# Zhen-Dong/HAWQ

Hardware: NVIDIA H100
Metric: images/sec ResNet-50 W8A8 & W4A4 @batch128, 1/2/4/8xH100; % int-TC roofline (higher is better)
Workload: dtype int8

## Files before the change

hawq_b200/csrc/conv_igemm.cuh:

```cuda
#pragma once
#include <type_traits>

#include "common.cuh"
#include "wgmma.cuh"

namespace hawq {

struct ConvParams {
  const uint8_t* x;
  const int8_t* w;
  const hawq_chan* chan;
  const void* res;
  const hawq_chan* res_chan;
  const float* fscale;
  void* out;
  void* out_low;
  int32_t* status;
  int N, H, W, Cin, Cout, KH, KW, stride, pad, Ho, Wo, M, K;
  int cin_chunks;
  int x_pix_bytes;
  int mode, relu, out_bits, lo, hi;
  int res_kind, res_bits;
  uint32_t res_m;
  int res_e;
  int y_bits, low_bits;
  uint32_t low_m;
  int low_e, low_lo, low_hi;
  int cout_store;
  int scalar_over_one;
  int scalar_unchecked;
  int check_ovf;
  int bias_lo, bias_hi;
  const uint8_t* x2;
  const int8_t* w2;
  int H2, W2, stride2, cin_chunks2, x2_pix_bytes;
};

constexpr int CONV_BM = 128;
constexpr int CONV_STAGES = 4;
constexpr int CONV_THREADS = 256;

template <int BN>
struct ChanSmem {
  static constexpr int M_OFF = BN * (int)sizeof(hawq_chan);
  static constexpr int M1_OFF = M_OFF + BN * 8;
  static constexpr int RC_OFF = M1_OFF + BN * 8;
  static constexpr int CB_OFF = RC_OFF + BN * (int)sizeof(hawq_chan);
  static constexpr int BYTES = CB_OFF + BN * 8;
  hawq_chan* chan;
  double* M;
  double* M1;
  hawq_chan* rc;
  double* Cb;
  __device__ explicit ChanSmem(uint8_t* base)
      : chan(reinterpret_cast<hawq_chan*>(base)), M(reinterpret_cast<double*>(base + M_OFF)),
        M1(reinterpret_cast<double*>(base + M1_OFF)), rc(reinterpret_cast<hawq_chan*>(base + RC_OFF)),
        Cb(reinterpret_cast<double*>(base + CB_OFF)) {}
};

template <int BN, bool A4>
struct ConvSmem {
  static constexpr int A_ROW = A4 ? 32 : 64;
  static constexpr int A_STAGE = CONV_BM * A_ROW;
  static constexpr int B_STAGE = BN * 64;
  static constexpr int PIPE = CONV_STAGES * (A_STAGE + B_STAGE);
  static constexpr int OUT_PITCH = BN + 16;
  static constexpr int OUT_STAGE = CONV_BM * OUT_PITCH;
  static constexpr int RES16 = CONV_BM * (BN * 2 + 16);
  static constexpr int RES32 = CONV_BM * (BN * 4 + 32);
  static constexpr int RES16_OFF = PIPE;
  static constexpr int RES32_OFF = OUT_STAGE;
  static constexpr int MAIN = PIPE + RES16 > RES32_OFF + RES32 ? PIPE + RES16 : RES32_OFF + RES32;
  static constexpr int CHAN_OFF = MAIN;
  static constexpr int TOTAL = CHAN_OFF + ChanSmem<BN>::BYTES;
  static_assert(OUT_STAGE <= PIPE, "the low-bit staging tile must fit in the freed ring");
  static_assert(2 * (TOTAL + 1024) <= 228 * 1024, "two CTAs per SM must fit in shared memory");
};

template <int ROW_BYTES>
__device__ __forceinline__ int swz(int row, int ch) {
  if constexpr (ROW_BYTES == 64) return row * 64 + ((ch ^ ((row >> 1) & 3)) << 4);
  else return row * 32 + ((ch ^ ((row >> 2) & 1)) << 4);
}

constexpr int FAM_REQUANT = 0, FAM_RESIDUAL = 1, FAM_STORE = 2, FAM_REQUANT_CAPPED = 3;

template <bool CLAMPED>
struct RqFp64 {
  bool checked;
  bool ovf = false;
  static constexpr double kMagic = 6755399441055744.0;
  __device__ static double acc_bias(int32_t acc, double cb, int32_t) {
    const double d = __hiloint2double(0x43300000, acc ^ 0x80000000) - cb;
    return CLAMPED ? fmin(fmax(d, -2147483648.0), 2147483647.0) : d;
  }
  __device__ static double of_i32(int32_t v) {
    return __hiloint2double(0x43300000, v ^ 0x80000000) - 4503601774854144.0;
  }
  __device__ static double of_u16(uint32_t u) { return __hiloint2double(0x43300000, (int)u) - 4503599627370496.0; }
  __device__ int32_t term(double d, double M, uint32_t, int32_t, bool count) {
    const double t = __fma_rn(d, M, kMagic);
    if (checked && count) {
      const double q = t - kMagic;
      ovf |= q > 2147483647.0 || q < -2147483648.0;
    }
    return __double2loint(t);
  }
};
struct RqExact {
  bool checked;
  bool ovf = false;
  __device__ static int32_t acc_bias(int32_t acc, double, int32_t bias) { return sat_add(acc, bias); }
  __device__ static int32_t of_i32(int32_t v) { return v; }
  __device__ static int32_t of_u16(uint32_t u) { return (int32_t)u; }
  __device__ int32_t term(int32_t v, double, uint32_t m, int32_t e, bool count) {
    const long long q = rhe_requant64(v, m, e);
    if (checked && count) ovf |= q > 2147483647ll || q < -2147483648ll;
    return sat_i32(q);
  }
};

struct RqPolicy {
  bool over_one;
  bool unchecked;
  bool clamped;
};

template <int BN, bool RESIDUAL, bool CAPS = false>
__device__ RqPolicy load_channel_block(const ConvParams& p, int n0, const ChanSmem<BN>& cs) {
  int over_one = p.scalar_over_one, unchecked = p.scalar_unchecked, bias_out = 0;
  const int tid = threadIdx.x;
  if (tid < BN) {
    hawq_chan c = p.chan[n0 + tid];
    if (CAPS) c.reserved = p.relu == 2 ? min(p.hi, c.reserved) : p.hi;
    cs.chan[tid] = c;
    cs.M[tid] = dyadic_to_double(c.m, c.e);
    cs.Cb[tid] = 4503601774854144.0 - (double)c.bias;
    bias_out = c.bias < p.bias_lo || c.bias > p.bias_hi;
    over_one |= !dyadic_is_fast(c.m, c.e);
    unchecked |= !dyadic_is_wide(c.m, c.e);
    if (RESIDUAL && p.res_kind == 1) {
      const hawq_chan rc = p.res_chan[n0 + tid];
      cs.rc[tid] = rc;
      cs.M1[tid] = dyadic_to_double(rc.m, rc.e);
      over_one |= !dyadic_is_fast(rc.m, rc.e);
      unchecked |= !dyadic_is_wide(rc.m, rc.e);
    }
  }
  RqPolicy pol;
  pol.over_one = __syncthreads_or(over_one) != 0;
  pol.unchecked = __syncthreads_or(unchecked) != 0;
  pol.clamped = __syncthreads_or(bias_out) != 0;
  return pol;
}

template <bool RESIDUAL, class F>
__device__ __forceinline__ void with_rq(const RqPolicy& pol, const ConvParams& p, F&& f) {
  const bool fp64 = !pol.over_one || (RESIDUAL && p.check_ovf && !pol.unchecked);
  if (!fp64) f(RqExact{RESIDUAL && p.check_ovf != 0});
  else if (pol.clamped) f(RqFp64<true>{RESIDUAL && pol.over_one});
  else f(RqFp64<false>{RESIDUAL && pol.over_one});
}

template <class Rq>
__device__ __forceinline__ int32_t residual_y(Rq& rq, int32_t res_term, int32_t acc, double cb, const int4& c, double M, bool ok,
                                              int32_t relu_floor) {
  return max(sat_add(res_term, rq.term(rq.acc_bias(acc, cb, c.x), M, c.y, c.z, ok)), relu_floor);
}
template <class Rq>
__device__ __forceinline__ int32_t residual_low(Rq& rq, int32_t y, double low_M, const ConvParams& p) {
  return clampi(rq.term(rq.of_i32(y), low_M, p.low_m, p.low_e, false), p.low_lo, p.low_hi);
}
__device__ __forceinline__ uint32_t stream16_pair(int32_t y0, int32_t y1, bool ok, int& ymax) {
  if (ok) ymax = max(ymax, max(y0, y1));
  return (uint32_t)min(y0, 65535) | ((uint32_t)min(y1, 65535) << 16);
}
__device__ __forceinline__ void residual_flags(const ConvParams& p, int ymax, bool ovf) {
  if (ymax > 65535) atomicOr(p.status, HAWQ_FLAG_RESIDUAL_OVERFLOW);
  if (ovf) atomicOr(p.status, HAWQ_FLAG_REQUANT_OVERFLOW);
}
__device__ __forceinline__ void stage_low_pair(uint8_t* s, int pitch, int row, int col, int q0, int q1) {
  *reinterpret_cast<uint16_t*>(s + row * pitch + col) = (uint16_t)__byte_perm(q0, q1, 0x0040);
}

__device__ __forceinline__ void copy_out_rows(const uint8_t* s, int s_pitch, uint8_t* g, size_t g_pitch, int row_bytes, int m0, int M) {
  const int cpr = row_bytes / 16;
  for (int id = threadIdx.x; id < CONV_BM * cpr; id += blockDim.x) {
    const int row = id / cpr, j = id - row * cpr;
    if (m0 + row < M)
      *reinterpret_cast<int4*>(g + (size_t)(m0 + row) * g_pitch + j * 16) = *reinterpret_cast<const int4*>(s + row * s_pitch + j * 16);
  }
}
template <int BN>
__device__ __forceinline__ void copy_out_low(const uint8_t* s, int pitch, uint8_t* gout, int bits, int m0, int n0, int M, int Cout) {
  if (bits == 8) {
    copy_out_rows(s, pitch, gout + n0, (size_t)Cout, BN, m0, M);
  } else {
    constexpr int CPR = BN / 32;
    for (int id = threadIdx.x; id < CONV_BM * CPR; id += blockDim.x) {
      const int row = id / CPR, j = id % CPR;
      if (m0 + row < M) {
        const uint4 a = *reinterpret_cast<const uint4*>(s + row * pitch + j * 32);
        const uint4 b = *reinterpret_cast<const uint4*>(s + row * pitch + j * 32 + 16);
        uint4 o;
        o.x = pack_nibbles8(a.x, a.y);
        o.y = pack_nibbles8(a.z, a.w);
        o.z = pack_nibbles8(b.x, b.y);
        o.w = pack_nibbles8(b.z, b.w);
        *reinterpret_cast<uint4*>(gout + (((size_t)(m0 + row) * Cout + n0 + j * 32) >> 1)) = o;
      }
    }
  }
}

struct ConvGeom {
  const uint8_t* x;
  const int8_t* w;
  int H, W, stride, pad, KH, KW, cin_chunks, x_pix_bytes, K;
};

template <int BN, bool A4, int FAM>
__global__ void __launch_bounds__(CONV_THREADS, 2) conv_igemm_kernel(const ConvParams p) {
  using S = ConvSmem<BN, A4>;
  constexpr int BM = CONV_BM, STAGES = CONV_STAGES;
  constexpr int A_ROW = S::A_ROW;
  constexpr int A_CH = A_ROW / 16;
  constexpr int A_ROWS_PER_PASS = CONV_THREADS / A_CH;
  constexpr int A_PASSES = BM / A_ROWS_PER_PASS;
  constexpr int B_PASSES = BN / 64;
  constexpr int NT = BN / 8;
  constexpr int NACC = BN / 2;

  extern __shared__ __align__(1024) uint8_t smem[];
  uint8_t* sA = smem;
  uint8_t* sB = smem + STAGES * S::A_STAGE;
  const ChanSmem<BN> cs(smem + S::CHAN_OFF);
  const hawq_chan* sChan = cs.chan;
  const double* sM = cs.M;
  const double* sM1 = cs.M1;
  const hawq_chan* sResChan = cs.rc;
  const double* sCb = cs.Cb;

  const int tid = threadIdx.x;
  const int lane = tid & 31, warp = tid >> 5;
  const int wg = warp >> 2;
  const int g = lane >> 2, t = lane & 3;
  const int nblk = p.Cout / BN;
  const int m0 = (int)(blockIdx.x / nblk) * BM;
  const int n0 = (int)(blockIdx.x % nblk) * BN;

  constexpr bool REQ = FAM == FAM_REQUANT || FAM == FAM_REQUANT_CAPPED;
  const RqPolicy pol = load_channel_block<BN, FAM == FAM_RESIDUAL, FAM == FAM_REQUANT_CAPPED>(p, n0, cs);

  int32_t acc[NACC];

  const int res_es = (FAM == FAM_RESIDUAL) ? ((p.res_kind == 1 || p.res_bits == 32) ? 4 : 2) : 0;
  const int res_pitch = BN * res_es + 8 * res_es;
  uint8_t* sRes = smem + (res_es == 2 ? S::RES16_OFF : S::RES32_OFF);

  auto load_res = [&]() {
    if constexpr (FAM == FAM_RESIDUAL) {
      const int cpr = BN * res_es / 16;
      const uint8_t* gres = reinterpret_cast<const uint8_t*>(p.res);
      for (int id = tid; id < BM * cpr; id += CONV_THREADS) {
        const int row = id / cpr, j = id - row * cpr;
        const bool v = m0 + row < p.M;
        const uint8_t* src = v ? gres + ((size_t)(m0 + row) * p.Cout + n0) * res_es + j * 16 : gres;
        cp_async_16(smem_u32(sRes + row * res_pitch + j * 16), src, v ? 16 : 0);
      }
    }
  };
  const bool prefetch_res = res_es == 2;

  auto gemm = [&](const ConvGeom& gm, bool with_res) {
#pragma unroll
    for (int i = 0; i < NACC; ++i) acc[i] = 0;
    const int a_ch = tid % A_CH;
    int a_hi0[A_PASSES], a_wi0[A_PASSES], a_pix[A_PASSES];
    bool a_ok[A_PASSES];
#pragma unroll
    for (int i = 0; i < A_PASSES; ++i) {
      const int row = tid / A_CH + i * A_ROWS_PER_PASS;
      const int m = m0 + row;
      a_ok[i] = m < p.M;
      const int mm = a_ok[i] ? m : 0;
      const int n = mm / (p.Ho * p.Wo);
      const int r = mm - n * (p.Ho * p.Wo);
      const int ho = r / p.Wo, wo = r - ho * p.Wo;
      a_hi0[i] = ho * gm.stride - gm.pad;
      a_wi0[i] = wo * gm.stride - gm.pad;
      a_pix[i] = n * gm.H * gm.W;
    }
    const int b_ch = tid & 3, b_row = tid >> 2;
    const int KT = gm.KH * gm.KW * gm.cin_chunks;
    int ld_c = 0, ld_kw = 0, ld_kh = 0, ld_kt = 0;

    auto load_tile = [&](int stage) {
      const uint32_t a_base = smem_u32(sA + stage * S::A_STAGE);
#pragma unroll
      for (int i = 0; i < A_PASSES; ++i) {
        const int row = tid / A_CH + i * A_ROWS_PER_PASS;
        const int hi = a_hi0[i] + ld_kh, wi = a_wi0[i] + ld_kw;
        const bool v = a_ok[i] && (unsigned)hi < (unsigned)gm.H && (unsigned)wi < (unsigned)gm.W;
        const uint8_t* src = gm.x;
        if (v) src = gm.x + (size_t)(a_pix[i] + hi * gm.W + wi) * gm.x_pix_bytes + ld_c * A_ROW + a_ch * 16;
        cp_async_16(a_base + swz<A_ROW>(row, a_ch), src, v ? 16 : 0);
      }
      const uint32_t b_base = smem_u32(sB + stage * S::B_STAGE);
#pragma unroll
      for (int i = 0; i < B_PASSES; ++i) {
        const int row = b_row + i * 64;
        const int8_t* src = gm.w + (size_t)(n0 + row) * gm.K + ld_kt * 64 + b_ch * 16;
        cp_async_16(b_base + swz<64>(row, b_ch), src, 16);
      }
      ++ld_kt;
      if (++ld_c == gm.cin_chunks) {
        ld_c = 0;
        if (++ld_kw == gm.KW) { ld_kw = 0; ++ld_kh; }
      }
    };

#pragma unroll
    for (int s = 0; s < STAGES - 1; ++s) {
      if (s < KT) load_tile(s);
      if (s == STAGES - 2 && with_res) load_res();
      cp_async_commit();
    }

    for (int kt = 0; kt < KT; ++kt) {
      cp_async_wait<STAGES - 2>();
      fence_proxy_async_smem();
      __syncthreads();
      if (kt + STAGES - 1 < KT) load_tile((kt + STAGES - 1) % STAGES);
      cp_async_commit();

      const int stage = kt % STAGES;
      const uint32_t a_base = smem_u32(sA + stage * S::A_STAGE);
      const uint32_t b_base = smem_u32(sB + stage * S::B_STAGE);
#pragma unroll
      for (int ks = 0; ks < 2; ++ks) {
        const uint64_t bdesc = wgmma_desc_sw64(b_base + ks * 32);
        if constexpr (!A4) {
          wgmma_fence();
          wgmma_ss<BN>(acc, wgmma_desc_sw64(a_base + wg * 64 * A_ROW + ks * 32), bdesc);
        } else {
          uint32_t r0, r1;
          const int row = warp * 16 + (lane & 7) + ((lane >> 3) & 1) * 8;
          ldmatrix_x2(r0, r1, a_base + swz<32>(row, ks));
          const uint32_t af[4] = {r0 & 0x0F0F0F0Fu, r1 & 0x0F0F0F0Fu, (r0 >> 4) & 0x0F0F0F0Fu, (r1 >> 4) & 0x0F0F0F0Fu};
          wgmma_fence();
          wgmma_rs<BN>(acc, af, bdesc);
        }
      }
      wgmma_commit();
      wgmma_wait_all();
      fence_operands(acc);
    }
    cp_async_wait<0>();
    __syncthreads();
  };

  gemm(ConvGeom{p.x, p.w, p.H, p.W, p.stride, p.pad, p.KH, p.KW, p.cin_chunks, p.x_pix_bytes, p.K}, prefetch_res);

  if (res_es == 4) {
    load_res();
    cp_async_commit();
    cp_async_wait<0>();
    __syncthreads();
  }
  const bool y_staged = res_es != 0 && p.y_bits == res_es * 8;
  const int y_es = p.y_bits / 8;
  const int y_pitch = BN * y_es + 8 * y_es;
  uint8_t* sY = sRes;

  uint8_t* sOut = smem;
  const bool stage_low = (REQ && p.out_bits <= 8) || (FAM == FAM_RESIDUAL && p.low_bits != 0);
  const int stage_bits = REQ ? p.out_bits : p.low_bits;

  auto put_low = [&](int row, int col, int q0, int q1) { stage_low_pair(sOut, S::OUT_PITCH, row, col, q0, q1); };
  auto put_y = [&](int row, int col, bool ok, int y0, int y1, int& ymax) {
    const uint32_t y16 = p.y_bits == 16 ? stream16_pair(y0, y1, ok, ymax) : 0u;
    if (!y_staged && !ok) return;
    uint8_t* dst = y_staged ? sY + row * y_pitch + col * y_es
                            : reinterpret_cast<uint8_t*>(p.out) + ((size_t)(m0 + row) * p.Cout + n0 + col) * y_es;
    if (p.y_bits == 16) *reinterpret_cast<uint32_t*>(dst) = y16;
    else if (p.y_bits == 32) *reinterpret_cast<int2*>(dst) = make_int2(y0, y1);
  };

  auto epilogue = [&](auto rq, auto low_out) {
    if constexpr (REQ) {
      const int lo = p.relu ? min(max(p.lo, 0), p.hi) : p.lo;
#pragma unroll
      for (int ni = 0; ni < NT; ++ni) {
        const int col = ni * 8 + 2 * t;
        const int4 c0 = *reinterpret_cast<const int4*>(&sChan[col]);
        const int4 c1 = *reinterpret_cast<const int4*>(&sChan[col + 1]);
        const double2 M = *reinterpret_cast<const double2*>(&sM[col]);
        const double2 Cb = *reinterpret_cast<const double2*>(&sCb[col]);
        const int hi0 = FAM == FAM_REQUANT_CAPPED ? c0.w : p.hi, hi1 = FAM == FAM_REQUANT_CAPPED ? c1.w : p.hi;
#pragma unroll
        for (int hf = 0; hf < 2; ++hf) {
          const int row = warp * 16 + hf * 8 + g;
          const int q0 = clampi(rq.term(rq.acc_bias(acc[ni * 4 + hf * 2], Cb.x, c0.x), M.x, c0.y, c0.z, false), lo, hi0);
          const int q1 = clampi(rq.term(rq.acc_bias(acc[ni * 4 + hf * 2 + 1], Cb.y, c1.x), M.y, c1.y, c1.z, false), lo, hi1);
          if constexpr (decltype(low_out)::value) {
            put_low(row, col, q0, q1);
          } else if (m0 + row < p.M) {
            uint8_t* dst = reinterpret_cast<uint8_t*>(p.out) + ((size_t)(m0 + row) * p.Cout + n0 + col) * (p.out_bits / 8);
            if (p.out_bits == 16) *reinterpret_cast<uint32_t*>(dst) = (uint32_t)(q0 & 0xFFFF) | ((uint32_t)q1 << 16);
            else *reinterpret_cast<int2*>(dst) = make_int2(q0, q1);
          }
        }
      }
    } else {
      const double res_M = dyadic_to_double(p.res_m, p.res_e), low_M = dyadic_to_double(p.low_m, p.low_e);
      const int relu_floor = p.relu ? 0 : (int)0x80000000;
      int ymax = 0;
#pragma unroll
      for (int ni = 0; ni < NT; ++ni) {
        const int col = ni * 8 + 2 * t;
        const int4 c0 = *reinterpret_cast<const int4*>(&sChan[col]);
        const int4 c1 = *reinterpret_cast<const int4*>(&sChan[col + 1]);
        const double2 M = *reinterpret_cast<const double2*>(&sM[col]);
        const double2 Cb = *reinterpret_cast<const double2*>(&sCb[col]);
        double2 M1 = make_double2(res_M, res_M);
        uint2 m1 = make_uint2(p.res_m, p.res_m);
        int2 e1 = make_int2(p.res_e, p.res_e);
        if (p.res_kind == 1) {
          M1 = *reinterpret_cast<const double2*>(&sM1[col]);
          m1 = make_uint2(sResChan[col].m, sResChan[col + 1].m);
          e1 = make_int2(sResChan[col].e, sResChan[col + 1].e);
        }
#pragma unroll
        for (int hf = 0; hf < 2; ++hf) {
          const int row = warp * 16 + hf * 8 + g;
          const bool ok = m0 + row < p.M;
          const uint8_t* rptr = sRes + row * res_pitch + col * res_es;
          decltype(rq.of_i32(0)) r0, r1;
          if (res_es == 2) {
            const uint32_t pr = *reinterpret_cast<const uint32_t*>(rptr);
            r0 = rq.of_u16(pr & 0xFFFFu);
            r1 = rq.of_u16(pr >> 16);
          } else {
            const int2 pr = *reinterpret_cast<const int2*>(rptr);
            r0 = rq.of_i32(pr.x);
            r1 = rq.of_i32(pr.y);
          }
          const int y0 = residual_y(rq, rq.term(r0, M1.x, m1.x, e1.x, ok), acc[ni * 4 + hf * 2 + 0], Cb.x, c0, M.x, ok, relu_floor);
          const int y1 = residual_y(rq, rq.term(r1, M1.y, m1.y, e1.y, ok), acc[ni * 4 + hf * 2 + 1], Cb.y, c1, M.y, ok, relu_floor);
          put_y(row, col, ok, y0, y1, ymax);
          if (p.low_bits != 0) put_low(row, col, residual_low(rq, y0, low_M, p), residual_low(rq, y1, low_M, p));
        }
      }
      residual_flags(p, ymax, rq.ovf);
    }
  };

  if constexpr (FAM == FAM_STORE) {
#pragma unroll
    for (int ni = 0; ni < NT; ++ni) {
      const int col = ni * 8 + 2 * t;
      const int b0 = sChan[col].bias, b1 = sChan[col + 1].bias;
#pragma unroll
      for (int hf = 0; hf < 2; ++hf) {
        const int m = m0 + warp * 16 + hf * 8 + g;
        if (m >= p.M) continue;
        const int32_t v0 = sat_add(acc[ni * 4 + hf * 2 + 0], b0), v1 = sat_add(acc[ni * 4 + hf * 2 + 1], b1);
        if (p.mode == HAWQ_EPI_RAW_I32) {
          *reinterpret_cast<int2*>(reinterpret_cast<int32_t*>(p.out) + (size_t)m * p.Cout + n0 + col) = make_int2(v0, v1);
        } else {
          float* o = reinterpret_cast<float*>(p.out) + (size_t)m * p.cout_store;
          const int c = n0 + col;
          if (c < p.cout_store) o[c] = __fmul_rn((float)v0, p.fscale[c]);
          if (c + 1 < p.cout_store) o[c + 1] = __fmul_rn((float)v1, p.fscale[c + 1]);
        }
      }
    }
  } else {
    auto run = [&](auto low_out) { with_rq<FAM == FAM_RESIDUAL>(pol, p, [&](auto rq) { epilogue(rq, low_out); }); };
    if (REQ && p.out_bits <= 8) run(std::true_type{});
    else run(std::false_type{});
  }

  if (y_staged || stage_low) __syncthreads();
  if (y_staged)
    copy_out_rows(sY, y_pitch, reinterpret_cast<uint8_t*>(p.out) + (size_t)n0 * y_es, (size_t)p.Cout * y_es, BN * y_es, m0, p.M);
  if (stage_low)
    copy_out_low<BN>(sOut, S::OUT_PITCH, reinterpret_cast<uint8_t*>(REQ ? p.out : p.out_low), stage_bits, m0, n0, p.M, p.Cout);
}

}
```

hawq_b200/csrc/conv_tail.cuh:

```cuda
#pragma once
#include "conv_igemm.cuh"

namespace hawq {

constexpr int TAIL_BN = 64;

template <bool A4, bool DUAL>
struct TailSmem {
  static constexpr int BN = TAIL_BN;
  static constexpr int A_ROW = A4 ? 32 : 64;
  static constexpr int A_STAGE = CONV_BM * A_ROW;
  static constexpr int B_STAGE = BN * 64;
  static constexpr int PIPE = CONV_STAGES * (A_STAGE + B_STAGE);
  static constexpr int Y_PITCH = BN * 2 + 16;
  static constexpr int Y_SLOT = CONV_BM * Y_PITCH;
  static constexpr int I_OFF = PIPE;
  static constexpr int Y_OFF = I_OFF + (DUAL ? BN / 4 * CONV_THREADS * 8 : 0);
  static constexpr int Y_SLOTS = DUAL ? 1 : 2;
  static constexpr int OUT_PITCH = BN + 16;
  static constexpr int OUT_OFF = Y_OFF + Y_SLOTS * Y_SLOT;
  static constexpr int CHAN_OFF = OUT_OFF + CONV_BM * OUT_PITCH;
  static constexpr int TOTAL = CHAN_OFF + ChanSmem<BN>::BYTES;
  static_assert(A_STAGE % 512 == 0 && B_STAGE % 512 == 0, "wgmma tiles must stay 512-B aligned");
  static_assert(Y_OFF % 16 == 0 && Y_SLOT % 16 == 0 && OUT_OFF % 16 == 0 && CHAN_OFF % 16 == 0, "16-byte copies need aligned tiles");
  static_assert(2 * (TOTAL + 1024) <= 228 * 1024, "two CTAs per SM must fit in shared memory");
};

inline int tail_grid(int Cout, int sm_count) {
  const int nblk = Cout / TAIL_BN;
  const int per = 2 * sm_count / nblk;
  return (per > 1 ? per : 1) * nblk;
}

template <bool A4, bool DUAL>
__global__ void __launch_bounds__(CONV_THREADS, 2) conv_tail_kernel(const ConvParams p) {
  using S = TailSmem<A4, DUAL>;
  constexpr int BN = TAIL_BN, BM = CONV_BM, STAGES = CONV_STAGES;
  constexpr int A_ROW = S::A_ROW;
  constexpr int A_CH = A_ROW / 16;
  constexpr int A_ROWS_PER_PASS = CONV_THREADS / A_CH;
  constexpr int A_PASSES = BM / A_ROWS_PER_PASS;
  constexpr int NT = BN / 8;
  constexpr int NACC = BN / 2;

  extern __shared__ __align__(1024) uint8_t smem[];
  uint8_t* sA = smem;
  uint8_t* sB = smem + STAGES * S::A_STAGE;
  uint8_t* sOut = smem + S::OUT_OFF;
  const ChanSmem<BN> cs(smem + S::CHAN_OFF);

  const int tid = threadIdx.x;
  const int lane = tid & 31, warp = tid >> 5;
  const int wg = warp >> 2;
  const int g = lane >> 2, t = lane & 3;

  const int nblk = p.Cout / BN;
  const int n0 = (int)(blockIdx.x % nblk) * BN;
  const int rt0 = (int)(blockIdx.x / nblk), rstep = (int)(gridDim.x / nblk);
  const int nrt = (p.M + BM - 1) / BM;
  if (rt0 >= nrt) return;
  const int T = (nrt - rt0 + rstep - 1) / rstep;

  const RqPolicy pol = load_channel_block<BN, true>(p, n0, cs);

  const int KT = p.cin_chunks;
  const int KT2 = DUAL ? p.cin_chunks2 : 0;
  const int KTT = KT + KT2;
  const int D = DUAL ? STAGES - 1 : min(STAGES - 1, KT);

  int ld_t = 0, ld_k = 0, ld_s = 0;
  int ld_pix2[A_PASSES];
  const int a_ch = tid % A_CH;
  const int b_ch = tid & 3, b_row = tid >> 2;
  auto issue = [&]() {
    if (ld_t < T) {
      const int lm0 = (rt0 + ld_t * rstep) * BM;
      const bool ident = DUAL && ld_k < KT2;
      const int kc = ident ? ld_k : ld_k - KT2;
      const uint8_t* xb = ident ? p.x2 : p.x;
      const int pix_bytes = ident ? p.x2_pix_bytes : p.x_pix_bytes;
      const uint32_t a_base = smem_u32(sA + ld_s * S::A_STAGE);
#pragma unroll
      for (int i = 0; i < A_PASSES; ++i) {
        const int row = tid / A_CH + i * A_ROWS_PER_PASS;
        const int m = lm0 + row;
        const bool v = m < p.M;
        if (DUAL && ld_k == 0 && v) {
          const int n = m / (p.Ho * p.Wo);
          const int r = m - n * (p.Ho * p.Wo);
          const int ho = r / p.Wo, wo = r - ho * p.Wo;
          ld_pix2[i] = (n * p.H2 + ho * p.stride2) * p.W2 + wo * p.stride2;
        }
        const uint8_t* src = xb;
        if (v) src = xb + (size_t)(ident ? ld_pix2[i] : m) * pix_bytes + kc * A_ROW + a_ch * 16;
        cp_async_16(a_base + swz<A_ROW>(row, a_ch), src, v ? 16 : 0);
      }
      const int8_t* wb = ident ? p.w2 : p.w;
      const int wk = (ident ? KT2 : KT) * 64;
      cp_async_16(smem_u32(sB + ld_s * S::B_STAGE) + swz<64>(b_row, b_ch), wb + (size_t)(n0 + b_row) * wk + kc * 64 + b_ch * 16, 16);
      if (!DUAL && ld_k == 0) {
        uint8_t* sr = smem + S::Y_OFF + (ld_t & 1) * S::Y_SLOT;
        const uint8_t* gres = reinterpret_cast<const uint8_t*>(p.res);
        constexpr int CPR = BN * 2 / 16;
        for (int id = tid; id < BM * CPR; id += CONV_THREADS) {
          const int row = id / CPR, j = id - row * CPR;
          const bool v = lm0 + row < p.M;
          const uint8_t* src = v ? gres + ((size_t)(lm0 + row) * p.Cout + n0) * 2 + j * 16 : gres;
          cp_async_16(smem_u32(sr + row * S::Y_PITCH + j * 16), src, v ? 16 : 0);
        }
      }
      if (++ld_k == KTT) { ld_k = 0; ++ld_t; }
      if (++ld_s == STAGES) ld_s = 0;
    }
    cp_async_commit();
  };

  int32_t acc[NACC];
  int cs_s = 0;
  auto consume = [&]() {
    if (D == 1) cp_async_wait<0>();
    else if (D == 2) cp_async_wait<1>();
    else cp_async_wait<2>();
    fence_proxy_async_smem();
    __syncthreads();
    issue();
    const uint32_t a_base = smem_u32(sA + cs_s * S::A_STAGE);
    const uint32_t b_base = smem_u32(sB + cs_s * S::B_STAGE);
    if (++cs_s == STAGES) cs_s = 0;
#pragma unroll
    for (int ks = 0; ks < 2; ++ks) {
      const uint64_t bdesc = wgmma_desc_sw64(b_base + ks * 32);
      if constexpr (!A4) {
        wgmma_fence();
        wgmma_ss<BN>(acc, wgmma_desc_sw64(a_base + wg * 64 * A_ROW + ks * 32), bdesc);
      } else {
        uint32_t r0, r1;
        const int row = warp * 16 + (lane & 7) + ((lane >> 3) & 1) * 8;
        ldmatrix_x2(r0, r1, a_base + swz<32>(row, ks));
        const uint32_t af[4] = {r0 & 0x0F0F0F0Fu, r1 & 0x0F0F0F0Fu, (r0 >> 4) & 0x0F0F0F0Fu, (r1 >> 4) & 0x0F0F0F0Fu};
        wgmma_fence();
        wgmma_rs<BN>(acc, af, bdesc);
      }
    }
    wgmma_commit();
    wgmma_wait_all();
    fence_operands(acc);
  };

  for (int s = 0; s < D; ++s) issue();

  const double res_M = dyadic_to_double(p.res_m, p.res_e), low_M = dyadic_to_double(p.low_m, p.low_e);
  const int relu_floor = p.relu ? 0 : (int)0x80000000;
  uint8_t* gy = reinterpret_cast<uint8_t*>(p.out) + (size_t)n0 * 2;

  with_rq<true>(pol, p, [&](auto rq) {
    int ymax = 0;
    for (int j = 0; j < T; ++j) {
      const int m0 = (rt0 + j * rstep) * BM;
      if constexpr (DUAL) {
#pragma unroll
        for (int i = 0; i < NACC; ++i) acc[i] = 0;
        for (int kt = 0; kt < KT2; ++kt) consume();
#pragma unroll
        for (int ni = 0; ni < NT; ++ni) {
          const int col = ni * 8 + 2 * t;
          const int4 r0 = *reinterpret_cast<const int4*>(&cs.rc[col]);
          const int4 r1 = *reinterpret_cast<const int4*>(&cs.rc[col + 1]);
          const double2 M1 = *reinterpret_cast<const double2*>(&cs.M1[col]);
#pragma unroll
          for (int hf = 0; hf < 2; ++hf) {
            const int row = warp * 16 + hf * 8 + g;
            const bool ok = m0 + row < p.M;
            const int i0 = ni * 4 + hf * 2;
            *reinterpret_cast<int2*>(smem + S::I_OFF + ((ni * 2 + hf) * CONV_THREADS + tid) * 8) =
                make_int2(rq.term(rq.of_i32(sat_add(acc[i0], r0.x)), M1.x, r0.y, r0.z, ok),
                          rq.term(rq.of_i32(sat_add(acc[i0 + 1], r1.x)), M1.y, r1.y, r1.z, ok));
          }
        }
      }
#pragma unroll
      for (int i = 0; i < NACC; ++i) acc[i] = 0;
      for (int kt = 0; kt < KT; ++kt) consume();

      uint8_t* sY = smem + S::Y_OFF + (DUAL ? 0 : (j & 1) * S::Y_SLOT);
#pragma unroll
      for (int ni = 0; ni < NT; ++ni) {
        const int col = ni * 8 + 2 * t;
        const int4 c0 = *reinterpret_cast<const int4*>(&cs.chan[col]);
        const int4 c1 = *reinterpret_cast<const int4*>(&cs.chan[col + 1]);
        const double2 M = *reinterpret_cast<const double2*>(&cs.M[col]);
        const double2 Cb = *reinterpret_cast<const double2*>(&cs.Cb[col]);
#pragma unroll
        for (int hf = 0; hf < 2; ++hf) {
          const int row = warp * 16 + hf * 8 + g;
          const bool ok = m0 + row < p.M;
          const int i0 = ni * 4 + hf * 2;
          uint32_t* yp = reinterpret_cast<uint32_t*>(sY + row * S::Y_PITCH + col * 2);
          int32_t t0, t1;
          if constexpr (DUAL) {
            const int2 it = *reinterpret_cast<const int2*>(smem + S::I_OFF + ((ni * 2 + hf) * CONV_THREADS + tid) * 8);
            t0 = it.x;
            t1 = it.y;
          } else {
            const uint32_t pr = *yp;
            t0 = rq.term(rq.of_u16(pr & 0xFFFFu), res_M, p.res_m, p.res_e, ok);
            t1 = rq.term(rq.of_u16(pr >> 16), res_M, p.res_m, p.res_e, ok);
          }
          const int y0 = residual_y(rq, t0, acc[i0], Cb.x, c0, M.x, ok, relu_floor);
          const int y1 = residual_y(rq, t1, acc[i0 + 1], Cb.y, c1, M.y, ok, relu_floor);
          *yp = stream16_pair(y0, y1, ok, ymax);
          if (p.low_bits != 0) stage_low_pair(sOut, S::OUT_PITCH, row, col, residual_low(rq, y0, low_M, p), residual_low(rq, y1, low_M, p));
        }
      }
      __syncthreads();
      copy_out_rows(sY, S::Y_PITCH, gy, (size_t)p.Cout * 2, BN * 2, m0, p.M);
      if (p.low_bits != 0) copy_out_low<BN>(sOut, S::OUT_PITCH, reinterpret_cast<uint8_t*>(p.out_low), p.low_bits, m0, n0, p.M, p.Cout);
    }
    residual_flags(p, ymax, rq.ovf);
  });
  cp_async_wait<0>();
}

}
```

hawq_b200/csrc/wgmma.cuh:

```cuda
#pragma once
#include "common.cuh"

namespace hawq {

__device__ __forceinline__ uint64_t wgmma_desc_sw64(uint32_t smem_addr) {
  return (uint64_t)((smem_addr >> 4) & 0x3FFFu) | ((uint64_t)1 << 16) | ((uint64_t)(512 >> 4) << 32) | ((uint64_t)2 << 62);
}
__device__ __forceinline__ void wgmma_fence() { asm volatile("wgmma.fence.sync.aligned;" ::: "memory"); }
__device__ __forceinline__ void wgmma_commit() { asm volatile("wgmma.commit_group.sync.aligned;" ::: "memory"); }
__device__ __forceinline__ void wgmma_wait_all() { asm volatile("wgmma.wait_group.sync.aligned 0;" ::: "memory"); }
__device__ __forceinline__ void fence_proxy_async_smem() { asm volatile("fence.proxy.async.shared::cta;" ::: "memory"); }
template <int N>
__device__ __forceinline__ void fence_operands(int32_t (&d)[N]) {
#pragma unroll
  for (int i = 0; i < N; ++i) asm volatile("" : "+r"(d[i])::"memory");
}

__device__ __forceinline__ void wgmma_ss_n64_s8(int32_t (&d)[32], uint64_t adesc, uint64_t bdesc) {
  asm volatile(
      "wgmma.mma_async.sync.aligned.m64n64k32.s32.s8.s8 "
      "{%0, %1, %2, %3, %4, %5, %6, %7, %8, %9, %10, %11, %12, %13, %14, %15, %16, %17, %18, %19, %20, %21, %22, %23, %24, %25, %26, %27, %28, %29, %30, %31}, "
      "%32, %33, 1;"
      : "+r"(d[0]), "+r"(d[1]), "+r"(d[2]), "+r"(d[3]), "+r"(d[4]), "+r"(d[5]), "+r"(d[6]), "+r"(d[7]), "+r"(d[8]), "+r"(d[9]), "+r"(d[10]), "+r"(d[11]), "+r"(d[12]), "+r"(d[13]), "+r"(d[14]), "+r"(d[15]), "+r"(d[16]), "+r"(d[17]), "+r"(d[18]), "+r"(d[19]), "+r"(d[20]), "+r"(d[21]), "+r"(d[22]), "+r"(d[23]), "+r"(d[24]), "+r"(d[25]), "+r"(d[26]), "+r"(d[27]), "+r"(d[28]), "+r"(d[29]), "+r"(d[30]), "+r"(d[31])
      : "l"(adesc), "l"(bdesc)
      : "memory");
}

__device__ __forceinline__ void wgmma_rs_n64_u8(int32_t (&d)[32], const uint32_t (&a)[4], uint64_t bdesc) {
  asm volatile(
      "wgmma.mma_async.sync.aligned.m64n64k32.s32.u8.s8 "
      "{%0, %1, %2, %3, %4, %5, %6, %7, %8, %9, %10, %11, %12, %13, %14, %15, %16, %17, %18, %19, %20, %21, %22, %23, %24, %25, %26, %27, %28, %29, %30, %31}, "
      "{%32, %33, %34, %35}, %36, 1;"
      : "+r"(d[0]), "+r"(d[1]), "+r"(d[2]), "+r"(d[3]), "+r"(d[4]), "+r"(d[5]), "+r"(d[6]), "+r"(d[7]), "+r"(d[8]), "+r"(d[9]), "+r"(d[10]), "+r"(d[11]), "+r"(d[12]), "+r"(d[13]), "+r"(d[14]), "+r"(d[15]), "+r"(d[16]), "+r"(d[17]), "+r"(d[18]), "+r"(d[19]), "+r"(d[20]), "+r"(d[21]), "+r"(d[22]), "+r"(d[23]), "+r"(d[24]), "+r"(d[25]), "+r"(d[26]), "+r"(d[27]), "+r"(d[28]), "+r"(d[29]), "+r"(d[30]), "+r"(d[31])
      : "r"(a[0]), "r"(a[1]), "r"(a[2]), "r"(a[3]), "l"(bdesc)
      : "memory");
}

__device__ __forceinline__ void wgmma_ss_n128_s8(int32_t (&d)[64], uint64_t adesc, uint64_t bdesc) {
  asm volatile(
      "wgmma.mma_async.sync.aligned.m64n128k32.s32.s8.s8 "
      "{%0, %1, %2, %3, %4, %5, %6, %7, %8, %9, %10, %11, %12, %13, %14, %15, %16, %17, %18, %19, %20, %21, %22, %23, %24, %25, %26, %27, %28, %29, %30, %31, %32, %33, %34, %35, %36, %37, %38, %39, %40, %41, %42, %43, %44, %45, %46, %47, %48, %49, %50, %51, %52, %53, %54, %55, %56, %57, %58, %59, %60, %61, %62, %63}, "
      "%64, %65, 1;"
      : "+r"(d[0]), "+r"(d[1]), "+r"(d[2]), "+r"(d[3]), "+r"(d[4]), "+r"(d[5]), "+r"(d[6]), "+r"(d[7]), "+r"(d[8]), "+r"(d[9]), "+r"(d[10]), "+r"(d[11]), "+r"(d[12]), "+r"(d[13]), "+r"(d[14]), "+r"(d[15]), "+r"(d[16]), "+r"(d[17]), "+r"(d[18]), "+r"(d[19]), "+r"(d[20]), "+r"(d[21]), "+r"(d[22]), "+r"(d[23]), "+r"(d[24]), "+r"(d[25]), "+r"(d[26]), "+r"(d[27]), "+r"(d[28]), "+r"(d[29]), "+r"(d[30]), "+r"(d[31]), "+r"(d[32]), "+r"(d[33]), "+r"(d[34]), "+r"(d[35]), "+r"(d[36]), "+r"(d[37]), "+r"(d[38]), "+r"(d[39]), "+r"(d[40]), "+r"(d[41]), "+r"(d[42]), "+r"(d[43]), "+r"(d[44]), "+r"(d[45]), "+r"(d[46]), "+r"(d[47]), "+r"(d[48]), "+r"(d[49]), "+r"(d[50]), "+r"(d[51]), "+r"(d[52]), "+r"(d[53]), "+r"(d[54]), "+r"(d[55]), "+r"(d[56]), "+r"(d[57]), "+r"(d[58]), "+r"(d[59]), "+r"(d[60]), "+r"(d[61]), "+r"(d[62]), "+r"(d[63])
      : "l"(adesc), "l"(bdesc)
      : "memory");
}

__device__ __forceinline__ void wgmma_rs_n128_u8(int32_t (&d)[64], const uint32_t (&a)[4], uint64_t bdesc) {
  asm volatile(
      "wgmma.mma_async.sync.aligned.m64n128k32.s32.u8.s8 "
      "{%0, %1, %2, %3, %4, %5, %6, %7, %8, %9, %10, %11, %12, %13, %14, %15, %16, %17, %18, %19, %20, %21, %22, %23, %24, %25, %26, %27, %28, %29, %30, %31, %32, %33, %34, %35, %36, %37, %38, %39, %40, %41, %42, %43, %44, %45, %46, %47, %48, %49, %50, %51, %52, %53, %54, %55, %56, %57, %58, %59, %60, %61, %62, %63}, "
      "{%64, %65, %66, %67}, %68, 1;"
      : "+r"(d[0]), "+r"(d[1]), "+r"(d[2]), "+r"(d[3]), "+r"(d[4]), "+r"(d[5]), "+r"(d[6]), "+r"(d[7]), "+r"(d[8]), "+r"(d[9]), "+r"(d[10]), "+r"(d[11]), "+r"(d[12]), "+r"(d[13]), "+r"(d[14]), "+r"(d[15]), "+r"(d[16]), "+r"(d[17]), "+r"(d[18]), "+r"(d[19]), "+r"(d[20]), "+r"(d[21]), "+r"(d[22]), "+r"(d[23]), "+r"(d[24]), "+r"(d[25]), "+r"(d[26]), "+r"(d[27]), "+r"(d[28]), "+r"(d[29]), "+r"(d[30]), "+r"(d[31]), "+r"(d[32]), "+r"(d[33]), "+r"(d[34]), "+r"(d[35]), "+r"(d[36]), "+r"(d[37]), "+r"(d[38]), "+r"(d[39]), "+r"(d[40]), "+r"(d[41]), "+r"(d[42]), "+r"(d[43]), "+r"(d[44]), "+r"(d[45]), "+r"(d[46]), "+r"(d[47]), "+r"(d[48]), "+r"(d[49]), "+r"(d[50]), "+r"(d[51]), "+r"(d[52]), "+r"(d[53]), "+r"(d[54]), "+r"(d[55]), "+r"(d[56]), "+r"(d[57]), "+r"(d[58]), "+r"(d[59]), "+r"(d[60]), "+r"(d[61]), "+r"(d[62]), "+r"(d[63])
      : "r"(a[0]), "r"(a[1]), "r"(a[2]), "r"(a[3]), "l"(bdesc)
      : "memory");
}

template <int N>
__device__ __forceinline__ void wgmma_ss(int32_t (&d)[N / 2], uint64_t adesc, uint64_t bdesc) {
  if constexpr (N == 128) wgmma_ss_n128_s8(d, adesc, bdesc);
  else wgmma_ss_n64_s8(d, adesc, bdesc);
}
template <int N>
__device__ __forceinline__ void wgmma_rs(int32_t (&d)[N / 2], const uint32_t (&a)[4], uint64_t bdesc) {
  if constexpr (N == 128) wgmma_rs_n128_u8(d, a, bdesc);
  else wgmma_rs_n64_u8(d, a, bdesc);
}

}
```

Measured before the change: 29140.

## Keep one wgmma group in flight and deepen pipeline for BN=64 convs

The conv implicit-GEMM main loop now waits for all but one committed wgmma group instead of draining every k-tile. It shortens the cp.async prefetch distance by one to keep the ring safe, and drains once after the loop. This applies to W8A8 multi-tap convs and to the dual tail kernel. BN=64 tiles get six stages instead of four, and the explicit accumulator zeroing is replaced by the wgmma scale-d predicate on the first k-step. The aim is to overlap tensor-core work with the next tile's sync and loads, at the cost of more shared memory per CTA and a shorter prefetch lookahead.

```diff
diff --git a/hawq_b200/csrc/conv_igemm.cuh b/hawq_b200/csrc/conv_igemm.cuh
--- a/hawq_b200/csrc/conv_igemm.cuh
+++ b/hawq_b200/csrc/conv_igemm.cuh
@@ -61,9 +61,10 @@
 template <int BN, bool A4>
 struct ConvSmem {
   static constexpr int A_ROW = A4 ? 32 : 64;
+  static constexpr int STAGES = BN == 64 ? 6 : CONV_STAGES;
   static constexpr int A_STAGE = CONV_BM * A_ROW;
   static constexpr int B_STAGE = BN * 64;
-  static constexpr int PIPE = CONV_STAGES * (A_STAGE + B_STAGE);
+  static constexpr int PIPE = STAGES * (A_STAGE + B_STAGE);
   static constexpr int OUT_PITCH = BN + 16;
   static constexpr int OUT_STAGE = CONV_BM * OUT_PITCH;
   static constexpr int RES16 = CONV_BM * (BN * 2 + 16);
@@ -222,7 +223,7 @@
 template <int BN, bool A4, int FAM>
 __global__ void __launch_bounds__(CONV_THREADS, 2) conv_igemm_kernel(const ConvParams p) {
   using S = ConvSmem<BN, A4>;
-  constexpr int BM = CONV_BM, STAGES = CONV_STAGES;
+  constexpr int BM = CONV_BM, STAGES = S::STAGES;
   constexpr int A_ROW = S::A_ROW;
   constexpr int A_CH = A_ROW / 16;
   constexpr int A_ROWS_PER_PASS = CONV_THREADS / A_CH;
@@ -273,8 +274,6 @@
   const bool prefetch_res = res_es == 2;
 
   auto gemm = [&](const ConvGeom& gm, bool with_res) {
-#pragma unroll
-    for (int i = 0; i < NACC; ++i) acc[i] = 0;
     const int a_ch = tid % A_CH;
     int a_hi0[A_PASSES], a_wi0[A_PASSES], a_pix[A_PASSES];
     bool a_ok[A_PASSES];
@@ -320,42 +319,51 @@
       }
     };
 
-#pragma unroll
-    for (int s = 0; s < STAGES - 1; ++s) {
-      if (s < KT) load_tile(s);
-      if (s == STAGES - 2 && with_res) load_res();
-      cp_async_commit();
-    }
-
-    for (int kt = 0; kt < KT; ++kt) {
-      cp_async_wait<STAGES - 2>();
-      fence_proxy_async_smem();
-      __syncthreads();
-      if (kt + STAGES - 1 < KT) load_tile((kt + STAGES - 1) % STAGES);
-      cp_async_commit();
-
-      const int stage = kt % STAGES;
-      const uint32_t a_base = smem_u32(sA + stage * S::A_STAGE);
-      const uint32_t b_base = smem_u32(sB + stage * S::B_STAGE);
-#pragma unroll
-      for (int ks = 0; ks < 2; ++ks) {
-        const uint64_t bdesc = wgmma_desc_sw64(b_base + ks * 32);
-        if constexpr (!A4) {
-          wgmma_fence();
-          wgmma_ss<BN>(acc, wgmma_desc_sw64(a_base + wg * 64 * A_ROW + ks * 32), bdesc);
-        } else {
-          uint32_t r0, r1;
-          const int row = warp * 16 + (lane & 7) + ((lane >> 3) & 1) * 8;
-          ldmatrix_x2(r0, r1, a_base + swz<32>(row, ks));
-          const uint32_t af[4] = {r0 & 0x0F0F0F0Fu, r1 & 0x0F0F0F0Fu, (r0 >> 4) & 0x0F0F0F0Fu, (r1 >> 4) & 0x0F0F0F0Fu};
-          wgmma_fence();
-          wgmma_rs<BN>(acc, af, bdesc);
+    auto kloop = [&](auto inflight) {
+      constexpr int INFLIGHT = decltype(inflight)::value;
+      constexpr int DIST = STAGES - 1 - INFLIGHT;
+#pragma unroll
+      for (int s = 0; s < DIST; ++s) {
+        if (s < KT) load_tile(s);
+        if (s == DIST - 1 && with_res) load_res();
+        cp_async_commit();
+      }
+
+      for (int kt = 0; kt < KT; ++kt) {
+        cp_async_wait<DIST - 1>();
+        fence_proxy_async_smem();
+        __syncthreads();
+        if (kt + DIST < KT) load_tile((kt + DIST) % STAGES);
+        cp_async_commit();
+
+        const int stage = kt % STAGES;
+        const uint32_t a_base = smem_u32(sA + stage * S::A_STAGE);
+        const uint32_t b_base = smem_u32(sB + stage * S::B_STAGE);
+#pragma unroll
+        for (int ks = 0; ks < 2; ++ks) {
+          const uint64_t bdesc = wgmma_desc_sw64(b_base + ks * 32);
+          const int accumulate = kt > 0 || ks > 0;
+          if constexpr (!A4) {
+            wgmma_fence();
+            wgmma_ss<BN>(acc, wgmma_desc_sw64(a_base + wg * 64 * A_ROW + ks * 32), bdesc, accumulate);
+          } else {
+            uint32_t r0, r1;
+            const int row = warp * 16 + (lane & 7) + ((lane >> 3) & 1) * 8;
+            ldmatrix_x2(r0, r1, a_base + swz<32>(row, ks));
+            const uint32_t af[4] = {r0 & 0x0F0F0F0Fu, r1 & 0x0F0F0F0Fu, (r0 >> 4) & 0x0F0F0F0Fu, (r1 >> 4) & 0x0F0F0F0Fu};
+            wgmma_fence();
+            wgmma_rs<BN>(acc, af, bdesc, accumulate);
+          }
         }
-      }
-      wgmma_commit();
-      wgmma_wait_all();
-      fence_operands(acc);
-    }
+        wgmma_commit();
+        wgmma_wait<INFLIGHT>();
+      }
+    };
+    if constexpr (A4) kloop(std::integral_constant<int, 0>{});
+    else if (gm.KH * gm.KW > 1) kloop(std::integral_constant<int, 1>{});
+    else kloop(std::integral_constant<int, 0>{});
+    wgmma_wait<0>();
+    fence_operands(acc);
     cp_async_wait<0>();
     __syncthreads();
   };
diff --git a/hawq_b200/csrc/conv_tail.cuh b/hawq_b200/csrc/conv_tail.cuh
--- a/hawq_b200/csrc/conv_tail.cuh
+++ b/hawq_b200/csrc/conv_tail.cuh
@@ -11,7 +11,8 @@
   static constexpr int A_ROW = A4 ? 32 : 64;
   static constexpr int A_STAGE = CONV_BM * A_ROW;
   static constexpr int B_STAGE = BN * 64;
-  static constexpr int PIPE = CONV_STAGES * (A_STAGE + B_STAGE);
+  static constexpr int STAGES = CONV_STAGES;
+  static constexpr int PIPE = STAGES * (A_STAGE + B_STAGE);
   static constexpr int Y_PITCH = BN * 2 + 16;
   static constexpr int Y_SLOT = CONV_BM * Y_PITCH;
   static constexpr int I_OFF = PIPE;
@@ -35,13 +36,14 @@
 template <bool A4, bool DUAL>
 __global__ void __launch_bounds__(CONV_THREADS, 2) conv_tail_kernel(const ConvParams p) {
   using S = TailSmem<A4, DUAL>;
-  constexpr int BN = TAIL_BN, BM = CONV_BM, STAGES = CONV_STAGES;
+  constexpr int BN = TAIL_BN, BM = CONV_BM, STAGES = S::STAGES;
   constexpr int A_ROW = S::A_ROW;
   constexpr int A_CH = A_ROW / 16;
   constexpr int A_ROWS_PER_PASS = CONV_THREADS / A_CH;
   constexpr int A_PASSES = BM / A_ROWS_PER_PASS;
   constexpr int NT = BN / 8;
   constexpr int NACC = BN / 2;
+  constexpr int INFLIGHT = DUAL && !A4 ? 1 : 0;
 
   extern __shared__ __align__(1024) uint8_t smem[];
   uint8_t* sA = smem;
@@ -66,7 +68,7 @@
   const int KT = p.cin_chunks;
   const int KT2 = DUAL ? p.cin_chunks2 : 0;
   const int KTT = KT + KT2;
-  const int D = DUAL ? STAGES - 1 : min(STAGES - 1, KT);
+  const int D = DUAL ? STAGES - 1 - INFLIGHT : min(STAGES - 1 - INFLIGHT, KT);
 
   int ld_t = 0, ld_k = 0, ld_s = 0;
   int ld_pix2[A_PASSES];
@@ -118,6 +120,7 @@
   int32_t acc[NACC];
   int cs_s = 0;
   auto consume = [&]() {
+    static_assert(STAGES - 1 - INFLIGHT <= 3, "consume() waits for at most three k-tiles ahead");
     if (D == 1) cp_async_wait<0>();
     else if (D == 2) cp_async_wait<1>();
     else cp_async_wait<2>();
@@ -132,18 +135,21 @@
       const uint64_t bdesc = wgmma_desc_sw64(b_base + ks * 32);
       if constexpr (!A4) {
         wgmma_fence();
-        wgmma_ss<BN>(acc, wgmma_desc_sw64(a_base + wg * 64 * A_ROW + ks * 32), bdesc);
+        wgmma_ss<BN>(acc, wgmma_desc_sw64(a_base + wg * 64 * A_ROW + ks * 32), bdesc, 1);
       } else {
         uint32_t r0, r1;
         const int row = warp * 16 + (lane & 7) + ((lane >> 3) & 1) * 8;
         ldmatrix_x2(r0, r1, a_base + swz<32>(row, ks));
         const uint32_t af[4] = {r0 & 0x0F0F0F0Fu, r1 & 0x0F0F0F0Fu, (r0 >> 4) & 0x0F0F0F0Fu, (r1 >> 4) & 0x0F0F0F0Fu};
         wgmma_fence();
-        wgmma_rs<BN>(acc, af, bdesc);
+        wgmma_rs<BN>(acc, af, bdesc, 1);
       }
     }
     wgmma_commit();
-    wgmma_wait_all();
+    wgmma_wait<INFLIGHT>();
+  };
+  auto drain = [&]() {
+    wgmma_wait<0>();
     fence_operands(acc);
   };
 
@@ -161,6 +167,7 @@
 #pragma unroll
         for (int i = 0; i < NACC; ++i) acc[i] = 0;
         for (int kt = 0; kt < KT2; ++kt) consume();
+        drain();
 #pragma unroll
         for (int ni = 0; ni < NT; ++ni) {
           const int col = ni * 8 + 2 * t;
@@ -181,6 +188,7 @@
 #pragma unroll
       for (int i = 0; i < NACC; ++i) acc[i] = 0;
       for (int kt = 0; kt < KT; ++kt) consume();
+      drain();
 
       uint8_t* sY = smem + S::Y_OFF + (DUAL ? 0 : (j & 1) * S::Y_SLOT);
 #pragma unroll
diff --git a/hawq_b200/csrc/wgmma.cuh b/hawq_b200/csrc/wgmma.cuh
--- a/hawq_b200/csrc/wgmma.cuh
+++ b/hawq_b200/csrc/wgmma.cuh
@@ -8,7 +8,8 @@
 }
 __device__ __forceinline__ void wgmma_fence() { asm volatile("wgmma.fence.sync.aligned;" ::: "memory"); }
 __device__ __forceinline__ void wgmma_commit() { asm volatile("wgmma.commit_group.sync.aligned;" ::: "memory"); }
-__device__ __forceinline__ void wgmma_wait_all() { asm volatile("wgmma.wait_group.sync.aligned 0;" ::: "memory"); }
+template <int N>
+__device__ __forceinline__ void wgmma_wait() { asm volatile("wgmma.wait_group.sync.aligned %0;" ::"n"(N) : "memory"); }
 __device__ __forceinline__ void fence_proxy_async_smem() { asm volatile("fence.proxy.async.shared::cta;" ::: "memory"); }
 template <int N>
 __device__ __forceinline__ void fence_operands(int32_t (&d)[N]) {
@@ -16,55 +17,59 @@
   for (int i = 0; i < N; ++i) asm volatile("" : "+r"(d[i])::"memory");
 }
 
-__device__ __forceinline__ void wgmma_ss_n64_s8(int32_t (&d)[32], uint64_t adesc, uint64_t bdesc) {
+__device__ __forceinline__ void wgmma_ss_n64_s8(int32_t (&d)[32], uint64_t adesc, uint64_t bdesc, int scale_d) {
   asm volatile(
+      "{\n.reg .pred p;\nsetp.ne.b32 p, %34, 0;\n"
       "wgmma.mma_async.sync.aligned.m64n64k32.s32.s8.s8 "
       "{%0, %1, %2, %3, %4, %5, %6, %7, %8, %9, %10, %11, %12, %13, %14, %15, %16, %17, %18, %19, %20, %21, %22, %23, %24, %25, %26, %27, %28, %29, %30, %31}, "
-      "%32, %33, 1;"
+      "%32, %33, p;\n}"
       : "+r"(d[0]), "+r"(d[1]), "+r"(d[2]), "+r"(d[3]), "+r"(d[4]), "+r"(d[5]), "+r"(d[6]), "+r"(d[7]), "+r"(d[8]), "+r"(d[9]), "+r"(d[10]), "+r"(d[11]), "+r"(d[12]), "+r"(d[13]), "+r"(d[14]), "+r"(d[15]), "+r"(d[16]), "+r"(d[17]), "+r"(d[18]), "+r"(d[19]), "+r"(d[20]), "+r"(d[21]), "+r"(d[22]), "+r"(d[23]), "+r"(d[24]), "+r"(d[25]), "+r"(d[26]), "+r"(d[27]), "+r"(d[28]), "+r"(d[29]), "+r"(d[30]), "+r"(d[31])
-      : "l"(adesc), "l"(bdesc)
+      : "l"(adesc), "l"(bdesc), "r"(scale_d)
       : "memory");
 }
 
-__device__ __forceinline__ void wgmma_rs_n64_u8(int32_t (&d)[32], const uint32_t (&a)[4], uint64_t bdesc) {
+__device__ __forceinline__ void wgmma_rs_n64_u8(int32_t (&d)[32], const uint32_t (&a)[4], uint64_t bdesc, int scale_d) {
   asm volatile(
+      "{\n.reg .pred p;\nsetp.ne.b32 p, %37, 0;\n"
       "wgmma.mma_async.sync.aligned.m64n64k32.s32.u8.s8 "
       "{%0, %1, %2, %3, %4, %5, %6, %7, %8, %9, %10, %11, %12, %13, %14, %15, %16, %17, %18, %19, %20, %21, %22, %23, %24, %25, %26, %27, %28, %29, %30, %31}, "
-      "{%32, %33, %34, %35}, %36, 1;"
+      "{%32, %33, %34, %35}, %36, p;\n}"
       : "+r"(d[0]), "+r"(d[1]), "+r"(d[2]), "+r"(d[3]), "+r"(d[4]), "+r"(d[5]), "+r"(d[6]), "+r"(d[7]), "+r"(d[8]), "+r"(d[9]), "+r"(d[10]), "+r"(d[11]), "+r"(d[12]), "+r"(d[13]), "+r"(d[14]), "+r"(d[15]), "+r"(d[16]), "+r"(d[17]), "+r"(d[18]), "+r"(d[19]), "+r"(d[20]), "+r"(d[21]), "+r"(d[22]), "+r"(d[23]), "+r"(d[24]), "+r"(d[25]), "+r"(d[26]), "+r"(d[27]), "+r"(d[28]), "+r"(d[29]), "+r"(d[30]), "+r"(d[31])
-      : "r"(a[0]), "r"(a[1]), "r"(a[2]), "r"(a[3]), "l"(bdesc)
+      : "r"(a[0]), "r"(a[1]), "r"(a[2]), "r"(a[3]), "l"(bdesc), "r"(scale_d)
       : "memory");
 }
 
-__device__ __forceinline__ void wgmma_ss_n128_s8(int32_t (&d)[64], uint64_t adesc, uint64_t bdesc) {
+__device__ __forceinline__ void wgmma_ss_n128_s8(int32_t (&d)[64], uint64_t adesc, uint64_t bdesc, int scale_d) {
   asm volatile(
+      "{\n.reg .pred p;\nsetp.ne.b32 p, %66, 0;\n"
       "wgmma.mma_async.sync.aligned.m64n128k32.s32.s8.s8 "
       "{%0, %1, %2, %3, %4, %5, %6, %7, %8, %9, %10, %11, %12, %13, %14, %15, %16, %17, %18, %19, %20, %21, %22, %23, %24, %25, %26, %27, %28, %29, %30, %31, %32, %33, %34, %35, %36, %37, %38, %39, %40, %41, %42, %43, %44, %45, %46, %47, %48, %49, %50, %51, %52, %53, %54, %55, %56, %57, %58, %59, %60, %61, %62, %63}, "
-      "%64, %65, 1;"
+      "%64, %65, p;\n}"
       : "+r"(d[0]), "+r"(d[1]), "+r"(d[2]), "+r"(d[3]), "+r"(d[4]), "+r"(d[5]), "+r"(d[6]), "+r"(d[7]), "+r"(d[8]), "+r"(d[9]), "+r"(d[10]), "+r"(d[11]), "+r"(d[12]), "+r"(d[13]), "+r"(d[14]), "+r"(d[15]), "+r"(d[16]), "+r"(d[17]), "+r"(d[18]), "+r"(d[19]), "+r"(d[20]), "+r"(d[21]), "+r"(d[22]), "+r"(d[23]), "+r"(d[24]), "+r"(d[25]), "+r"(d[26]), "+r"(d[27]), "+r"(d[28]), "+r"(d[29]), "+r"(d[30]), "+r"(d[31]), "+r"(d[32]), "+r"(d[33]), "+r"(d[34]), "+r"(d[35]), "+r"(d[36]), "+r"(d[37]), "+r"(d[38]), "+r"(d[39]), "+r"(d[40]), "+r"(d[41]), "+r"(d[42]), "+r"(d[43]), "+r"(d[44]), "+r"(d[45]), "+r"(d[46]), "+r"(d[47]), "+r"(d[48]), "+r"(d[49]), "+r"(d[50]), "+r"(d[51]), "+r"(d[52]), "+r"(d[53]), "+r"(d[54]), "+r"(d[55]), "+r"(d[56]), "+r"(d[57]), "+r"(d[58]), "+r"(d[59]), "+r"(d[60]), "+r"(d[61]), "+r"(d[62]), "+r"(d[63])
-      : "l"(adesc), "l"(bdesc)
+      : "l"(adesc), "l"(bdesc), "r"(scale_d)
       : "memory");
 }
 
-__device__ __forceinline__ void wgmma_rs_n128_u8(int32_t (&d)[64], const uint32_t (&a)[4], uint64_t bdesc) {
+__device__ __forceinline__ void wgmma_rs_n128_u8(int32_t (&d)[64], const uint32_t (&a)[4], uint64_t bdesc, int scale_d) {
   asm volatile(
+      "{\n.reg .pred p;\nsetp.ne.b32 p, %69, 0;\n"
       "wgmma.mma_async.sync.aligned.m64n128k32.s32.u8.s8 "
       "{%0, %1, %2, %3, %4, %5, %6, %7, %8, %9, %10, %11, %12, %13, %14, %15, %16, %17, %18, %19, %20, %21, %22, %23, %24, %25, %26, %27, %28, %29, %30, %31, %32, %33, %34, %35, %36, %37, %38, %39, %40, %41, %42, %43, %44, %45, %46, %47, %48, %49, %50, %51, %52, %53, %54, %55, %56, %57, %58, %59, %60, %61, %62, %63}, "
-      "{%64, %65, %66, %67}, %68, 1;"
+      "{%64, %65, %66, %67}, %68, p;\n}"
       : "+r"(d[0]), "+r"(d[1]), "+r"(d[2]), "+r"(d[3]), "+r"(d[4]), "+r"(d[5]), "+r"(d[6]), "+r"(d[7]), "+r"(d[8]), "+r"(d[9]), "+r"(d[10]), "+r"(d[11]), "+r"(d[12]), "+r"(d[13]), "+r"(d[14]), "+r"(d[15]), "+r"(d[16]), "+r"(d[17]), "+r"(d[18]), "+r"(d[19]), "+r"(d[20]), "+r"(d[21]), "+r"(d[22]), "+r"(d[23]), "+r"(d[24]), "+r"(d[25]), "+r"(d[26]), "+r"(d[27]), "+r"(d[28]), "+r"(d[29]), "+r"(d[30]), "+r"(d[31]), "+r"(d[32]), "+r"(d[33]), "+r"(d[34]), "+r"(d[35]), "+r"(d[36]), "+r"(d[37]), "+r"(d[38]), "+r"(d[39]), "+r"(d[40]), "+r"(d[41]), "+r"(d[42]), "+r"(d[43]), "+r"(d[44]), "+r"(d[45]), "+r"(d[46]), "+r"(d[47]), "+r"(d[48]), "+r"(d[49]), "+r"(d[50]), "+r"(d[51]), "+r"(d[52]), "+r"(d[53]), "+r"(d[54]), "+r"(d[55]), "+r"(d[56]), "+r"(d[57]), "+r"(d[58]), "+r"(d[59]), "+r"(d[60]), "+r"(d[61]), "+r"(d[62]), "+r"(d[63])
-      : "r"(a[0]), "r"(a[1]), "r"(a[2]), "r"(a[3]), "l"(bdesc)
+      : "r"(a[0]), "r"(a[1]), "r"(a[2]), "r"(a[3]), "l"(bdesc), "r"(scale_d)
       : "memory");
 }
 
 template <int N>
-__device__ __forceinline__ void wgmma_ss(int32_t (&d)[N / 2], uint64_t adesc, uint64_t bdesc) {
-  if constexpr (N == 128) wgmma_ss_n128_s8(d, adesc, bdesc);
-  else wgmma_ss_n64_s8(d, adesc, bdesc);
+__device__ __forceinline__ void wgmma_ss(int32_t (&d)[N / 2], uint64_t adesc, uint64_t bdesc, int scale_d) {
+  if constexpr (N == 128) wgmma_ss_n128_s8(d, adesc, bdesc, scale_d);
+  else wgmma_ss_n64_s8(d, adesc, bdesc, scale_d);
 }
 template <int N>
-__device__ __forceinline__ void wgmma_rs(int32_t (&d)[N / 2], const uint32_t (&a)[4], uint64_t bdesc) {
-  if constexpr (N == 128) wgmma_rs_n128_u8(d, a, bdesc);
-  else wgmma_rs_n64_u8(d, a, bdesc);
+__device__ __forceinline__ void wgmma_rs(int32_t (&d)[N / 2], const uint32_t (&a)[4], uint64_t bdesc, int scale_d) {
+  if constexpr (N == 128) wgmma_rs_n128_u8(d, a, bdesc, scale_d);
+  else wgmma_rs_n64_u8(d, a, bdesc, scale_d);
 }
 
 }
```

Result: no change. 29440, median of 6 (+1.0%).
